# fzaiser/genfer

Hardware: AMD Instinct MI355X
Metric: TaylorPoly mul f64 GMAC/s (higher is better)
Workload: dtype f64

## Files before the change

### genfer_amd/__init__.py

```python
from __future__ import annotations

import ctypes
import os

os.environ.setdefault("HIP_FORCE_DEV_KERNARG", "1")

from . import series
from . import interval_series
from .taylor import USIZE_MAX, TaylorError, bind

_HERE = os.path.dirname(os.path.abspath(__file__))
LIB_PATH = os.path.join(_HERE, "csrc", "libgftaylor.so")

_lib = None
_classes = {}


def lib() -> ctypes.CDLL:
    global _lib
    if _lib is None:
        if not os.path.exists(LIB_PATH):
            raise ImportError(
                f"{LIB_PATH} is missing — build it with `make -C genfer_amd/csrc` "
                "(or `python -c 'import __graft_entry__ as g; g.build()'`). There is no CPU fallback."
# ... 86 lines not shown
    out, tj = ctypes.c_void_p(), ctypes.c_void_p()
    rc = H.gfh_run(source.encode(), flags.encode(), backend_lib.encode(), prefix.encode(), ctypes.byref(out), ctypes.byref(tj))
    text = ctypes.string_at(out).decode() if out else ""
    timings = json.loads(ctypes.string_at(tj).decode()) if tj else None
    if out:
        H.gfh_free(out)
    if tj:
        H.gfh_free(tj)
    return rc, text, timings


def run_sgcl(source: str, flags: str = ""):
    lib()
    prefix = "gfti_" if any(t in ("-b", "--bounds") for t in flags.split()) else "gft_"
    rc, text, timings = run_sgcl_with_backend(source, flags, LIB_PATH, prefix)
    if rc != 0:
        raise TaylorError(text)
    return text, timings


OP_STATS = ("linear_scans", "scalar_readbacks", "coefficient_readbacks", "tiled", "staged", "per_output", "host_tier_ops",
            "host_to_device_mirrors")
OP_STATS_EX = ("launches", "deferred_ops", "chains_materialised", "chain_addsub_launches", "launches_in_place", "shallow_products",
               "fused_horner_steps", "tiled_peeled", "unused_8", "riders", "fused_observe_adds", "scans_proven", "nested_adds",
               "graph_executions", "graph_recordings", "batch_launches", "batch_items", "graph_us")


def pool_stats() -> dict:
    a = (ctypes.c_size_t * 3)()
    lib().gft_pool_stats(a)
    return {"in_use": int(a[0]), "cached": int(a[1]), "peak": int(a[2])}


def op_stats() -> dict:
    L = lib()
    a, b = (ctypes.c_size_t * 8)(), (ctypes.c_size_t * 32)()
    L.gft_op_stats(a)
    n = min(L.gft_op_stats_ex(b, 32), 32)
    out = dict(zip(OP_STATS, (int(v) for v in a)))
    out.update(dict(zip(OP_STATS_EX, (int(v) for v in b[:n]))))
    return out


def _sz(seq):
    seq = [int(s) for s in seq]
    return (ctypes.c_size_t * max(len(seq), 1))(*seq)

# ... 41 lines not shown
```

### genfer_amd/csrc/gft_api.hip

```cpp
#include <hip/hip_runtime.h>
#include <dlfcn.h>
#include <rccl/rccl.h>

#include <algorithm>
#include <chrono>
#include <atomic>
#include <cmath>
#include <cstdio>
#include <cstring>
#include <deque>
#include <exception>
#include <functional>
#include <initializer_list>
#include <map>
#include <memory>
#include <tuple>
#include <stdexcept>
#include <string>
#include <vector>

#include "../../include/gftaylor.h"
#include "gft_kernels.hpp"
#include "gft_small_alloc.hpp"
#include "gft_host.hpp"
// ... 121 lines not shown
typedef SmallVecT<size_t> Dims;
typedef SmallVecT<long long> Shifts;

namespace {

struct Error : std::runtime_error {
    using std::runtime_error::runtime_error;
};

thread_local std::string g_err;

#define HIP_OK(call)                                                                                  \
    do {                                                                                              \
        hipError_t e_ = (call);                                                                       \
        if (e_ != hipSuccess)                                                                         \
            throw Error(std::string("HIP error: ") + hipGetErrorString(e_) + " in " #call);           \
    } while (0)

struct Runtime {
    bool ready = false;
    int device = -1;
    hipStream_t own_stream = nullptr;
    hipStream_t stream = nullptr;
    size_t stats_peeled = 0;
    size_t stats_side[4] = {0, 0, 0, 0};
    size_t stats_nz = 0;
    size_t stats_sum = 0;
    bool lazy_sum = true;
    bool nz_proofs = true;
    bool lazy_horner = true;
    bool batch_dag = true;
    bool lazy_observe = true;
    hipStream_t side = nullptr;
    hipEvent_t ev_main = nullptr, ev_bulk = nullptr;
    bool side_pending = false;
    bool recur_overlap = true;
    std::map<size_t, std::vector<void*>> free_blocks;
    size_t in_use = 0, cached = 0, peak = 0;
    size_t peak_total = 0;
    unsigned* d_flag = nullptr;
    double* d_scratch = nullptr;
    unsigned* d_wit = nullptr;
    double* h_pinned = nullptr;
    double* h_mail = nullptr;
    double* d_mail = nullptr;
    unsigned long long mail_seq = 0;
// ... 1035 lines not shown
    return guard_int([&] {
        HIP_OK(hipStreamSynchronize(R.stream));
        R.stream = s ? (hipStream_t)s : R.own_stream;
        return 0;
    });
}
void* gft_get_stream(void) { return (void*)R.stream; }
int gft_device(void) {
    return guard_int([&] { return R.device; });
}
int gft_synchronize(void) {
    return guard_int([&] {
        HIP_OK(hipStreamSynchronize(R.stream));
        return 0;
    });
}
const char* gft_last_error(void) { return g_err.c_str(); }
const char* gfti_last_error(void) { return g_err.c_str(); }
void gft_op_stats(size_t out[8]) {
    for (int i = 0; i < 8; ++i) out[i] = R.stats[i];
}
size_t gft_op_stats_ex(size_t* out, size_t cap) {
    const size_t v[18] = {(size_t)gft::g_launches, R.stats_ex[0], R.stats_ex[1], R.stats_ex[2], (size_t)gft::g_launches_in_place,
                          R.stats_shallow[0], R.stats_shallow[1], R.stats_peeled, R.stats_side[1], R.stats_side[2], R.stats_side[3], R.stats_nz, R.stats_sum,
                          g_dag_stats[0], g_dag_stats[1], g_dag_stats[2], g_dag_stats[3], g_dag_stats[4]};
    for (size_t i = 0; i < 18 && i < cap; ++i) out[i] = v[i];
    return 18;
}
void gft_pool_stats(size_t out[3]) {
    const size_t ws = staged_scratch_bytes() + R.conv_ws_bytes;
    out[0] = R.in_use + ws;
    out[1] = R.cached;
    R.peak_total = std::max(R.peak_total, R.in_use + ws);
    out[2] = R.peak_total;
}
int gft_event_record(int slot) {
    return guard_int([&] {
        if (slot < 0 || slot >= 64) throw Error("event slot out of range");
        HIP_OK(hipEventRecord(R.events[slot], R.stream));
        return 0;
    });
}
float gft_event_elapsed_ms(int a, int b) {
    try {
        require_ready();
        if (a < 0 || a >= 64 || b < 0 || b >= 64) throw Error("event slot out of range");
        HIP_OK(hipEventSynchronize(R.events[b]));
// ... 9 lines not shown
    std::string n = name ? name : "";
    if (n == "horner_loop_max") R.horner_loop_max = value < 0 ? 0 : (size_t)value;
    else if (n == "div_wavefront") R.div_wavefront = value != 0;
    else if (n == "exp_right") R.exp_right = value != 0;
    else if (n == "recur_overlap") R.recur_overlap = value != 0;
    else if (n == "defer") R.defer = value != 0;
    else if (n == "lazy_observe") R.lazy_observe = value != 0;
    else if (n == "batch_dag") R.batch_dag = value != 0;
    else if (n == "lazy_horner") R.lazy_horner = value != 0;
    else if (n == "nz_proofs") R.nz_proofs = value != 0;
    else if (n == "lazy_sum") R.lazy_sum = value != 0;
    else if (n == "async_launch") lq_configure(R.device, value != 0);
    else if (n == "trace_lq_report") lq_report();
    else if (n == "shallow_max_terms") R.shallow_max_terms = value < 0 ? 256 : (size_t)value;
    else if (n == "debug_fail_next_launch") g_fail_next_launch.store(value != 0 ? 1 : 0);
    else if (n == "tiled_min_macs") R.tiled_min_macs = value;
    else if (n == "conv_rb_min_macs") staged_set_rb_min_macs(value);
    else if (n == "conv_rb_pairs") staged_set_rb_pairs(value);
    else if (n == "conv_rb_pairs_cap") staged_set_rb_pairs_cap(value);
    else if (n == "conv_rb_pairs_lanes") staged_set_rb_pairs_lanes(value);
    else if (n == "shallow_pair_min") shallow_set_pair_min(value == -1.0 ? 4096.0 : value);
    else if (n == "tiled_tile") tiled_set_lane_tile((int)value);
    else if (n == "tiled_peel") tiled_set_peel((int)value);
    else if (n == "host_max_elems") R.host_max_elems = value < 0 ? Runtime::HOST_MAX_ELEMS_DEFAULT : (size_t)value;
    else if (n == "host_max_macs") R.host_max_macs = value < 0 ? Runtime::HOST_MAX_MACS_DEFAULT : value;
    else if (n == "series_form") R.series_force = (value == 1 || value == 2) ? (int)value : 0;
    else if (n == "dist_min_macs") dist_set_min_macs(value);
    else if (n == "dist_event_slot") dist_set_event_slot(value);
    else return -1;
    return 0;
}
int gft_set_conv_variant(int v) {
    R.conv_variant = v;
    return 0;
}
int gft_set_conv_mode(int mode) {
    if (mode < 0 || mode > 3) return -1;
    R.conv_mode = mode;
    return 0;
}

int gft_conv_raw(const double* x, const size_t* xshape, const double* y, const size_t* yshape, double* res,
                 const size_t* rshape, size_t ndim, size_t slab_lo, size_t slab_hi, int accumulate) {
    return guard_int([&] {
        typedef Ops<EF64> O;
        O::HV xv{const_cast<double*>(x), 0, dims(xshape, ndim)};
// ... 574 lines not shown
```

### genfer_amd/csrc/gft_conv_tiled.hip

```cpp
#include <algorithm>
#include <cstdlib>
#include <cstring>
#include <map>
#include <vector>

#include "gft_kernels.hpp"

namespace gft {

namespace {

struct TileSeg {
    unsigned u, a, b;
    unsigned step_begin, step_end;
    int dest;
};

struct RedTile {
    unsigned u, a, b;
    unsigned first, count;
    unsigned slot0;
};

struct TiledArgs {
    unsigned xU, x0, x1, xI;
    unsigned yU, y0, y1, yI;
    unsigned zU, z0, z1, zI;
    unsigned nx8, ny8;
    unsigned nxc, nyc, nb;
    unsigned P1;
    unsigned tsh;
    unsigned slab_axis;
    unsigned slab_lo, slab_hi;
    int accumulate;
    unsigned xcd_remap;
    unsigned cut;
    unsigned lim1;
    size_t zsU, zs0, zs1, zoff;
    const double* xp;
    const double* yp;
    double* z;
    double* ws;
    const TileSeg* segs;
    const unsigned* wg_begin;
    const RedTile* red;
    const unsigned* red_slots;
    const unsigned* guard;
    unsigned guard_epoch;
    unsigned char blk1[8], blk2[8];
};

typedef const double __attribute__((address_space(4))) * cptr_t;

#ifndef GFT_TILED_DEFAULT_VARIANT
// ... 175 lines not shown
    unsigned julo, n_ju, j0lo, n_j0, j1lo, n_j1;
};

__host__ __device__ inline TileGeom tile_geom(const TiledArgs& A, unsigned tsh, unsigned u, unsigned a, unsigned b) {
    TileGeom g;
    const unsigned T0 = 64u >> tsh, T1 = 1u << tsh;
    g.julo = (u + 1 > A.yU) ? (u + 1 - A.yU) : 0;
    unsigned juhi = (u + 1 < A.xU) ? (u + 1) : A.xU;
    g.n_ju = juhi > g.julo ? juhi - g.julo : 0;
    unsigned k0max = (T0 * a + T0 - 1 < A.z0 - 1) ? T0 * a + T0 - 1 : A.z0 - 1;
    g.j0lo = (T0 * a + 1 > A.y0) ? (T0 * a + 1 - A.y0) : 0;
    unsigned j0hi = (k0max + 1 < A.x0) ? (k0max + 1) : A.x0;
    if ((A.cut & 1u) && T0 * a + 1 < j0hi) j0hi = T0 * a + 1;
    g.n_j0 = j0hi > g.j0lo ? j0hi - g.j0lo : 0;
    unsigned k1max = (T1 * b + T1 - 1 < A.z1 - 1) ? T1 * b + T1 - 1 : A.z1 - 1;
    g.j1lo = (T1 * b + 1 > A.y1) ? (T1 * b + 1 - A.y1) : 0;
    unsigned j1hi = (k1max + 1 < A.x1) ? (k1max + 1) : A.x1;
    if ((A.cut & 2u) && T1 * b + 1 < j1hi) j1hi = T1 * b + 1;
    g.n_j1 = j1hi > g.j1lo ? j1hi - g.j1lo : 0;
    return g;
}

constexpr unsigned YPAD = 8;


template <int NW, int VAR, int TSH>
__global__ void __launch_bounds__(NW * 64, 4)
k_conv_tiled(TiledArgs A) {
    constexpr bool FAST = (VAR & 1) != 0;
    constexpr bool NO_WINDOW = (VAR & 64) != 0;
    constexpr bool PEEL = (VAR & 128) != 0;
    extern __shared__ double lds[];
    if (A.guard && *A.guard == A.guard_epoch) return;
    const unsigned tid = threadIdx.x;
    const unsigned lane = tid & 63u;
    const unsigned wave = __builtin_amdgcn_readfirstlane(tid >> 6);
    const unsigned tsh = TSH ? (unsigned)TSH : A.tsh, T1m = (1u << tsh) - 1u, T0 = 64u >> tsh;
    const unsigned l0 = lane >> tsh, l1 = lane & T1m;
    constexpr unsigned NT = NW * 64;

    const unsigned c1 = A.blk1[wave];
    const unsigned c2 = A.blk2[wave];
    const bool has1 = c1 != 0xffu;
    const bool has2 = c2 != 0xffu;

    const unsigned half_row = A.ny8 >> 1;
    const unsigned hr_magic = (1u << 24) / half_row + 1u;
    const size_t y_row_stride = A.ny8;
    const unsigned pf_s0 = (tid * hr_magic) >> 24, pf_col = tid - pf_s0 * half_row;
    const bool pf_mine = pf_s0 < T0;
    double* const lds_lane = lds + (size_t)(l0 << tsh) * A.P1 + YPAD;
    double* const lds_pf = lds + (size_t)(pf_s0 << tsh) * A.P1 + YPAD + 2 * pf_col;

    unsigned wg = blockIdx.x;
    if (A.xcd_remap) wg = (blockIdx.x & 7u) * (gridDim.x >> 3) + (blockIdx.x >> 3);
    const unsigned seg_begin = A.wg_begin[wg], seg_end = A.wg_begin[wg + 1];
    for (unsigned si = seg_begin; si < seg_end; ++si) {
        const TileSeg seg = A.segs[si];
        const unsigned u = seg.u, a = seg.a, b = seg.b;
        const TileGeom g = tile_geom(A, tsh, u, a, b);
        const unsigned k0 = T0 * a + l0, k1 = (b << tsh) + l1;
        bool lane_in = k0 < A.z0 && k1 < A.z1;
        if (A.slab_axis == 1) lane_in = lane_in && k0 >= A.slab_lo && k0 < A.slab_hi;
        else if (A.slab_axis == 2) lane_in = lane_in && k1 >= A.slab_lo && k1 < A.slab_hi;
        unsigned y1lim = A.y1;
        if (PEEL && A.lim1 && (k1 & ~7u) + 1u < y1lim) y1lim = (k1 & ~7u) + 1u;

        double acc1[8], acc2[8];
#pragma unroll
        for (int i = 0; i < 8; ++i) acc1[i] = acc2[i] = 0.0;

        unsigned tj1 = seg.step_begin % g.n_j1;
        unsigned t = seg.step_begin / g.n_j1;
        unsigned tj0 = t % g.n_j0;
        unsigned ju = g.julo + t / g.n_j0, j0 = g.j0lo + tj0, j1 = g.j1lo + tj1;
        unsigned steps_left = seg.step_end - seg.step_begin;
        const unsigned j1_end = g.j1lo + g.n_j1;

        while (steps_left) {
            const unsigned row_steps = steps_left < j1_end - j1 ? steps_left : j1_end - j1;
            const double* ybase = A.yp + (size_t)(u - ju) * A.y0 * A.y1 * y_row_stride;
            if (!NO_WINDOW) {
                __syncthreads();
                for (unsigned p = tid; p < 64 * half_row; p += NT) {
                    unsigned row = (p * hr_magic) >> 24, col = p - row * half_row;
                    unsigned s0 = row >> tsh, s1 = row & T1m;
                    int R0 = (int)(T0 * a + s0) - (int)j0;
                    int R1 = (int)((b << tsh) + s1) - (int)j1;
                    if (R0 >= 0 && R0 < (int)A.y0 && R1 >= 0 && R1 < (int)A.y1) {
                        const double2 v = *reinterpret_cast<const double2*>(
                            ybase + ((size_t)R0 * A.y1 + (size_t)R1) * y_row_stride + 2 * col);
                        double* d = lds + ((s0 << tsh) + ((unsigned)R1 & T1m)) * A.P1 + YPAD + 2 * col;
                        d[0] = v.x;
                        d[1] = v.y;
                    }
                }
                __syncthreads();
            }
            cptr_t xr = (cptr_t)(A.xp + (((size_t)ju * A.x0 + j0) * A.x1 + j1) * A.nx8);
            const bool valid0 = lane_in && j0 <= k0 && (k0 - j0) < A.y0;
            int d1 = (int)k1 - (int)j1;
            int R1n = (int)(b << tsh) - (int)j1 - 1;
            const int pf_R0 = (int)(T0 * a + pf_s0) - (int)j0;
            const bool pf_row = pf_mine && pf_R0 >= 0 && pf_R0 < (int)A.y0;
            const double* pf_src = ybase + ((ptrdiff_t)pf_R0 * (ptrdiff_t)A.y1 + R1n) * (ptrdiff_t)y_row_stride + 2 * pf_col;

            for (unsigned rs = row_steps; rs > 0; --rs) {
                const bool last = rs == 1;
                const bool do_pf = !NO_WINDOW && !last && R1n >= 0 && R1n < (int)A.y1;
                double2 pf;
                if (do_pf && pf_row) pf = *reinterpret_cast<const double2*>(pf_src);

                if (valid0 && (unsigned)d1 < (PEEL ? y1lim : A.y1)) {
                    const double* yrow = lds_lane + (size_t)((unsigned)d1 & T1m) * A.P1;
                    if constexpr (FAST && (VAR & 8)) {
                        if (has1) block_fast_gen<VAR>(acc1, c1, xr, yrow, A.nxc, A.nyc);
                        if (has2) block_fast_gen<VAR>(acc2, c2, xr, yrow, A.nxc, A.nyc);
                    } else if constexpr (FAST) {
                        if (has1) block_fast<VAR>(acc1, c1, xr, yrow);
                        if (has2) block_fast<VAR>(acc2, c2, xr, yrow);
                    } else {
                        if (has1) block_mac<VAR>(acc1, c1, xr, yrow, A.nxc, A.nyc);
                        if (has2) block_mac<VAR>(acc2, c2, xr, yrow, A.nxc, A.nyc);
                    }
                }

                if (!last && !NO_WINDOW) {
                    __syncthreads();
                    if (do_pf && pf_row) {
                        double* d = lds_pf + (size_t)((unsigned)R1n & T1m) * A.P1;
                        d[0] = pf.x;
                        d[1] = pf.y;
                    }
                    __syncthreads();
                }
                xr += A.nx8;
                d1 -= 1;
                R1n -= 1;
                pf_src -= y_row_stride;
            }
            steps_left -= row_steps;
            j1 = g.j1lo;
            if (j0 + 1 < g.j0lo + g.n_j0) j0++;
            else {
                j0 = g.j0lo;
                ju++;
            }
        }

        if (seg.dest < 0) {
            if (lane_in) {
                double* zrow = A.z + (((size_t)u * A.z0 + k0) * A.z1 + k1) * A.zI;
                if constexpr (PEEL) zrow = A.z + A.zoff + (size_t)u * A.zsU + (size_t)k0 * A.zs0 + (size_t)k1 * A.zs1;
                if (has1) {
#pragma unroll
                    for (int r = 0; r < 8; ++r) {
                        unsigned k2 = 8 * c1 + r;
                        if (k2 < A.zI) zrow[k2] = A.accumulate ? zrow[k2] + acc1[r] : acc1[r];
                    }
                }
                if (has2) {
// ... 251 lines not shown
    plan_cache().clear();
    plan_generation()++;
    arena().head = 0;
}

int num_cus() {
    static int n = 0;
    if (!n) {
        int dev = 0;
        (void)hipGetDevice(&dev);
        hipDeviceProp_t p;
        if (hipGetDeviceProperties(&p, dev) == hipSuccess) n = p.multiProcessorCount;
        if (n <= 0) n = 256;
    }
    return n;
}

struct PeelSpec {
    unsigned role = 0;
    unsigned cut = 0, lim1 = 0;
    size_t zsU = 0, zs0 = 0, zs1 = 0, zoff = 0;
};

int& tiled_force_tsh() {
    static int v = 0;
    return v;
}

unsigned pick_lane_tile(const TiledArgs& T) {
    auto axis_eff = [](unsigned T, unsigned nx, unsigned ny, unsigned nz) {
        double useful = 0, issued = 0;
        for (unsigned t = 0; t * T < nz; ++t) {
            const unsigned kmax = std::min(T * t + T - 1, nz - 1);
            const unsigned jlo = T * t + 1 > ny ? T * t + 1 - ny : 0, jhi = std::min(kmax + 1, nx);
            if (jhi > jlo) issued += (double)(jhi - jlo) * T;
            for (unsigned k = T * t; k <= kmax; ++k) {
                const unsigned lo = k + 1 > ny ? k + 1 - ny : 0, hi = std::min(k + 1, nx);
                if (hi > lo) useful += hi - lo;
            }
        }
        return issued > 0 ? useful / issued : 0.0;
    };
    const int force = tiled_force_tsh();
    if (force >= 3 && force <= 6) return (unsigned)force;
    double best = -1.0;
    unsigned best_tsh = 3;
// ... 20 lines not shown
    }
    auto cost = [&](unsigned c) {
        unsigned n = 0;
        for (unsigned xc = 0; xc <= c && xc < T.nxc; ++xc)
            if (c - xc < T.nyc) n++;
        return n;
    };
    unsigned simd_load[4] = {0, 0, 0, 0}, wave_load[8] = {0}, wave_cnt[8] = {0};
    for (unsigned i = 0; i < T.nb; ++i) {
        unsigned c = T.nb - 1 - i;
        int best = -1;
        for (unsigned w = 0; w < NW; ++w) {
            if (wave_cnt[w] >= 2) continue;
            if (best < 0) { best = (int)w; continue; }
            unsigned sb = simd_load[best % 4], sw = simd_load[w % 4];
            if (sw < sb || (sw == sb && wave_load[w] < wave_load[best])) best = (int)w;
        }
        if (wave_cnt[best] == 0) T.blk1[best] = (unsigned char)c;
        else T.blk2[best] = (unsigned char)c;
        wave_cnt[best]++;
        wave_load[best] += cost(c);
        simd_load[best % 4] += cost(c);
    }
}

bool canonicalise(const ConvArgs& a, const Variant& V, const PeelSpec& ps, Plan& P) {
    TiledArgs& T = P.base;
    std::memset(&T, 0, sizeof(T));
    if (a.slab_axis < 0 || a.slab_axis >= a.nd - 1) return false;
    if (a.nd == 2) {
        T.xU = T.yU = T.zU = 1;
        T.x0 = T.y0 = T.z0 = 1;
        T.x1 = a.xs[0]; T.xI = a.xs[1];
        T.y1 = a.ys[0]; T.yI = a.ys[1];
        T.z1 = a.zs[0]; T.zI = a.zs[1];
        T.slab_axis = 2;
    } else if (a.nd == 3) {
        T.xU = T.yU = T.zU = 1;
        T.x0 = a.xs[0]; T.x1 = a.xs[1]; T.xI = a.xs[2];
        T.y0 = a.ys[0]; T.y1 = a.ys[1]; T.yI = a.ys[2];
        T.z0 = a.zs[0]; T.z1 = a.zs[1]; T.zI = a.zs[2];
        T.slab_axis = 1 + (unsigned)a.slab_axis;
    } else if (a.nd == 4) {
        T.xU = a.xs[0]; T.x0 = a.xs[1]; T.x1 = a.xs[2]; T.xI = a.xs[3];
        T.yU = a.ys[0]; T.y0 = a.ys[1]; T.y1 = a.ys[2]; T.yI = a.ys[3];
        T.zU = a.zs[0]; T.z0 = a.zs[1]; T.z1 = a.zs[2]; T.zI = a.zs[3];
// ... 2 lines not shown
        return false;
    }
    if (T.zI > 128 || T.xI > T.zI || T.yI > T.zI) return false;
    if (a.j0_min != 0 || a.j0_excl != 0 || a.j0_desc != 0) return false;
    T.nx8 = (T.xI + 7) / 8 * 8;
    T.ny8 = (T.yI + 7) / 8 * 8;
    T.nxc = T.nx8 / 8;
    T.nyc = T.ny8 / 8;
    T.nb = (T.zI + 7) / 8;
    T.P1 = V.b128 ? T.ny8 + YPAD + 2 : T.ny8 + YPAD + 1;
    T.tsh = pick_lane_tile(T);
    T.cut = ps.cut;
    T.lim1 = ps.lim1;
    if (ps.role >= 2) {
        T.zsU = ps.zsU; T.zs0 = ps.zs0; T.zs1 = ps.zs1; T.zoff = ps.zoff;
    } else {
        T.zsU = (size_t)T.z0 * T.z1 * T.zI; T.zs0 = (size_t)T.z1 * T.zI; T.zs1 = T.zI; T.zoff = 0;
    }
    T.slab_lo = a.slab_lo;
    T.slab_hi = a.slab_hi;
    T.accumulate = a.accumulate;
    unsigned npairs = (T.nb + 1) / 2;
    P.NW = npairs <= 1 ? 1 : (npairs <= 2 ? 2 : (npairs <= 4 ? 4 : 8));
    P.lds_bytes = (size_t)64 * T.P1 * sizeof(double);
    assign_blocks(T, P.NW);
    return true;
}

struct PlanTables {
    std::vector<TileSeg> segs;
    std::vector<unsigned> wg_begin;
    std::vector<RedTile> red;
    std::vector<unsigned> red_slots;
    bool slots_consecutive = true;
};

bool cut_ranges(Plan& P, PlanTables& tb) {
    const TiledArgs& T = P.base;
    const unsigned TT0 = 64u >> T.tsh, TT1 = 1u << T.tsh;
    struct TileInfo { unsigned u, a, b; unsigned long long steps; };
    std::vector<TileInfo> tiles;
    unsigned u_lo = 0, u_hi = T.zU, a_lo = 0, a_hi = (T.z0 + TT0 - 1) / TT0, b_lo = 0, b_hi = (T.z1 + TT1 - 1) / TT1;
    if (T.slab_axis == 0) {
        u_lo = T.slab_lo;
        u_hi = T.slab_hi;
    } else if (T.slab_axis == 1) {
        a_lo = T.slab_lo / TT0;
        a_hi = (T.slab_hi + TT0 - 1) / TT0;
    } else {
        b_lo = T.slab_lo / TT1;
        b_hi = (T.slab_hi + TT1 - 1) / TT1;
    }
    unsigned long long S = 0;
    for (unsigned u = u_lo; u < u_hi; ++u)
        for (unsigned aa = a_lo; aa < a_hi; ++aa)
            for (unsigned bb = b_lo; bb < b_hi; ++bb) {
                TileGeom g = tile_geom(T, T.tsh, u, aa, bb);
                unsigned long long st = (unsigned long long)g.n_ju * g.n_j0 * g.n_j1;
                if (st == 0 || st > 0xffffffffull) return false;
                tiles.push_back({u, aa, bb, st});
                S += st;
            }
    if (tiles.empty()) return false;
    unsigned wg_per_cu = std::min<unsigned>(16u / P.NW, (unsigned)(160 * 1024 / P.lds_bytes));
    if (wg_per_cu < 1) wg_per_cu = 1;
    unsigned long long n_wg = (unsigned long long)num_cus() * wg_per_cu;
    const unsigned long long per_slot = S / n_wg;
    const unsigned long long fit = per_slot / 190;
    n_wg *= fit >= 8 ? 8u : (fit >= 4 ? 4u : (fit >= 2 ? 2u : 1u));
    constexpr unsigned long long MIN_UNITS = 64;
    const unsigned long long step_units = (unsigned long long)T.nb * (T.nb + 1) / 2 + 3;
    const unsigned long long min_steps =
        std::max<unsigned long long>(1, (MIN_UNITS + 20ull * T.nb + step_units / 2) / step_units);
    if (n_wg > S / min_steps) n_wg = std::max<unsigned long long>(1, S / min_steps);
    P.n_wg = (unsigned)n_wg;

    tb.wg_begin.assign(P.n_wg + 1, 0);
    std::vector<std::vector<unsigned>> tile_slots(tiles.size());
    std::vector<int> tile_direct(tiles.size(), 0);
    unsigned n_slots = 0;
    size_t ti = 0;
    unsigned long long tile_start = 0;
    for (unsigned w = 0; w < P.n_wg; ++w) {
        unsigned long long lo = S * w / n_wg, hi = S * (w + 1) / n_wg;
        tb.wg_begin[w] = (unsigned)tb.segs.size();
        unsigned long long pos = lo;
        while (pos < hi) {
            while (pos >= tile_start + tiles[ti].steps) {
// ... 54 lines not shown
        }
        off += al(bytes);
        return d;
    };
    T.segs = (const TileSeg*)put(tb.segs.data(), b_segs);
    T.wg_begin = (const unsigned*)put(tb.wg_begin.data(), b_wg);
    T.red = (const RedTile*)put(tb.red.data(), b_red);
    T.red_slots = (const unsigned*)put(tb.red_slots.data(), b_rs);
    if (tb.slots_consecutive) T.red_slots = nullptr;
    if (hbase && hipMemcpyAsync(base, hbase, off, hipMemcpyHostToDevice, st) != hipSuccess) return false;
    return true;
}

bool build_plan(const ConvArgs& a, const Variant& V, const PeelSpec& ps, Plan& P, hipStream_t st) {
    PlanTables tb;
    return canonicalise(a, V, ps, P) && cut_ranges(P, tb) && upload_tables(P, tb, st);
}

template <int NW, int VAR, int TSH>
void launch_main_t(hipStream_t st, const Plan& P, const TiledArgs& T) {
    static bool attr_set = false;
    if (!attr_set) {
        (void)hipFuncSetAttribute(reinterpret_cast<const void*>(&k_conv_tiled<NW, VAR, TSH>),
                                  hipFuncAttributeMaxDynamicSharedMemorySize, 160 * 1024);
        attr_set = true;
    }
    GFT_LAUNCH((k_conv_tiled<NW, VAR, TSH>), dim3(P.n_wg), dim3(NW * 64), P.lds_bytes, st, T);
}
template <int NW, int VAR>
void launch_main_nw(hipStream_t st, const Plan& P, const TiledArgs& T) {
    if (T.tsh == 3) launch_main_t<NW, VAR, 3>(st, P, T);
    else launch_main_t<NW, VAR, 0>(st, P, T);
}
template <int VAR>
void launch_main(hipStream_t st, const Plan& P, const TiledArgs& T) {
    switch (P.NW) {
        case 1: launch_main_nw<1, VAR>(st, P, T); break;
        case 2: launch_main_nw<2, VAR>(st, P, T); break;
        case 4: launch_main_nw<4, VAR>(st, P, T); break;
        default: launch_main_nw<8, VAR>(st, P, T); break;
    }
}

}

void tiled_pad_rows_f64(hipStream_t st, const double* in, double* out, size_t rows, unsigned len, unsigned P, unsigned B) {
    size_t tot = rows * P * B;
// ... 2 lines not shown
                       len, P, B);
}
void tiled_fold_rows_f64(hipStream_t st, const double* zt, double* z, size_t rows, size_t row_lo, size_t row_hi, unsigned Pz,
                         unsigned B, unsigned zI, int accumulate, const unsigned* guard, unsigned epoch) {
    size_t tot = (row_hi - row_lo) * zI;
    if (!tot) return;
    GFT_LAUNCH(k_fold_rows, dim3((unsigned)std::min<size_t>((tot + 255) / 256, 4096)), dim3(256), 0, st, zt, z, rows,
                       row_lo, row_hi, Pz, B, zI, accumulate, guard, epoch);
}

void tiled_set_lane_tile(int tsh) { tiled_force_tsh() = tsh; }

namespace {

int& tiled_peel_mode() {
    static int v = GFT_TILED_PEEL_DEFAULT;
    return v;
}

const Plan* cached_plan(const ConvArgs& a, const Variant& V, const PeelSpec& ps, hipStream_t st) {
    PlanKey key;
    std::memset(&key, 0, sizeof(key));
    if (a.nd < 2 || a.nd > 4) return nullptr;
    key.v[0] = (unsigned)a.nd | ((unsigned)a.slab_axis << 8) | ((unsigned)tiled_force_tsh() << 16);
    for (int i = 0; i < a.nd; ++i) {
        key.v[1 + i] = a.xs[i];
        key.v[5 + i] = a.ys[i];
        key.v[9 + i] = a.zs[i];
    }
    key.v[13] = a.slab_lo;
    key.v[14] = a.slab_hi;
    key.v[15] = (unsigned)a.accumulate;
    key.v[16] = (unsigned)(a.j0_min | (a.j0_excl << 8) | (a.j0_desc << 16));
    key.v[17] = V.b128;
    key.v[18] = ps.role | (ps.cut << 4) | (ps.lim1 << 8);
    auto& cache = plan_cache();
    auto it = cache.find(key);
    if (it == cache.end()) {
        Plan P;
        if (cache.size() >= 1024) reset_plan_cache(st);
        if (!build_plan(a, V, ps, P, st)) return nullptr;
        it = cache.emplace(key, P).first;
    }
    return &it->second;
}

bool launch_plan(hipStream_t st, const Plan& P, TiledArgs T, const Variant& V) {
// ... 55 lines not shown
    T.guard = nf_flag;
    T.guard_epoch = nf_epoch;
}

bool peel_applies(const ConvArgs& a, const Variant& V) {
    const int mode = tiled_peel_mode();
    if (mode == 0) return false;
    if (a.nd != 3 || a.slab_axis != 0 || a.slab_lo != 0 || a.slab_hi != a.zs[0]) return false;
    if (a.j0_min || a.j0_excl || a.j0_desc) return false;
    for (int i = 0; i < 3; ++i)
        if (a.xs[i] != a.zs[i] || a.ys[i] != a.zs[i]) return false;
    const unsigned n0 = a.zs[0], n1 = a.zs[1];
    if (n0 % 8 || n1 % 8 || n0 < 16 || n1 < 16 || a.zs[2] > 128) return false;
    if (!V.fast || !V.b128 || V.compact || V.peel || V.other) return false;
    TiledArgs T;
    std::memset(&T, 0, sizeof(T));
    T.x0 = T.y0 = T.z0 = n0;
    T.x1 = T.y1 = T.z1 = n1;
    if (pick_lane_tile(T) != 3) return false;
    return mode == 1 || (n0 >= PEEL_MIN_EXTENT && n1 >= PEEL_MIN_EXTENT && a.zs[2] >= PEEL_MIN_INNER);
}

int conv_tiled_peel(hipStream_t st, const double* x, const double* y, double* z, const ConvArgs& a, const Variant& V, void* ws,
                    size_t ws_bytes, size_t* ws_needed, unsigned* nf_flag, unsigned nf_epoch, bool* guarded) {
    const unsigned n0 = a.zs[0], n1 = a.zs[1], nI = a.zs[2];
    ConvArgs l0, l1;
    std::memset(&l0, 0, sizeof(l0));
    l0.nd = 4;
    l0.slab_lo = 0;
    l0.slab_hi = 7;
    l0.accumulate = 1;
    l1 = l0;
    Variant VL = V;
    VL.peel = true;
    const unsigned s0x[4] = {7, 1, n1, nI}, s0y[4] = {7, n0 / 8, n1, nI}, s1x[4] = {7, 1, n0, nI}, s1y[4] = {7, n1 / 8, n0, nI};
    for (int i = 0; i < 4; ++i) {
        l0.xs[i] = s0x[i]; l0.ys[i] = l0.zs[i] = s0y[i];
        l1.xs[i] = s1x[i]; l1.ys[i] = l1.zs[i] = s1y[i];
    }
    PeelSpec pm, p0, p1;
    pm.role = 1; pm.cut = 3;
    p0.role = 2; p0.zsU = (size_t)n1 * nI; p0.zs0 = 8 * p0.zsU; p0.zs1 = nI; p0.zoff = p0.zsU;
    p1.role = 3; p1.lim1 = 1; p1.zsU = nI; p1.zs0 = 8 * (size_t)nI; p1.zs1 = (size_t)n1 * nI; p1.zoff = nI;
    Plan PM, P0, P1;
    for (int attempt = 0;; ++attempt) {
        const unsigned long long gen = plan_generation();
        const Plan* q = cached_plan(a, V, pm, st);
        if (!q) return -1;
        PM = *q;
        if (!(q = cached_plan(l0, VL, p0, st))) return -1;
        P0 = *q;
        if (!(q = cached_plan(l1, VL, p1, st))) return -1;
        P1 = *q;
        if (gen == plan_generation()) break;
        if (attempt) return -1;
    }
    const TiledArgs& B = PM.base;
    if (B.tsh != 3) return -1;
    const size_t n8 = B.nx8;
    const Operands o = operand_layout(B, std::max(PM.n_slots, std::max(P0.n_slots, P1.n_slots)), x, y, a.operands_slack);
    const size_t e_w0 = (size_t)7 * (n0 / 8) * n1 * n8, e_s1 = (size_t)7 * n0 * n8, e_w1 = (size_t)7 * (n1 / 8) * n0 * n8;
    auto al = [](size_t v) { return (v + 255) / 256 * 256; };
    const size_t o_w0 = o.end, o_s1 = o_w0 + al(e_w0 * sizeof(double)), o_w1 = o_s1 + al((e_s1 + 8) * sizeof(double)),
                 need = o_w1 + al(e_w1 * sizeof(double)) + 256;
    if (ws && ws_bytes < need) return -1;
    if (ws_needed) *ws_needed = need;
    if (guarded) *guarded = !o.inplace;
    if (!ws) return 1;

    char* wb = (char*)ws;
    double *w0 = (double*)(wb + o_w0), *s1 = (double*)(wb + o_s1), *w1 = (double*)(wb + o_w1);
    TiledArgs T = B;
    bind_operands(st, o, x, y, wb, nf_flag, nf_epoch, T);
    {
        const size_t tot = e_w0 + e_s1 + e_w1;
        GFT_LAUNCH(k_pack_peel, dim3((unsigned)std::min<size_t>((tot + 255) / 256, 4096)), dim3(256), 0, st, x, y, w0, s1, w1, n0, n1,
                   nI, (unsigned)n8);
    }
    T.z = z;
    if (!launch_plan(st, PM, T, V)) return 0;
    TiledArgs T0 = P0.base, T1 = P1.base;
    T0.ws = T1.ws = T.ws;
    T0.z = T1.z = z;
    T0.guard = T1.guard = T.guard;
    T0.guard_epoch = T1.guard_epoch = T.guard_epoch;
    T0.xp = T.yp;
    T0.yp = w0;
    T1.xp = s1;
    T1.yp = w1;
    return launch_plan(st, P0, T0, VL) && launch_plan(st, P1, T1, VL) ? 1 : 0;
}

}

void tiled_set_peel(int mode) { tiled_peel_mode() = mode < 0 ? -1 : (mode ? 1 : 0); }

bool conv_tiled_f64(hipStream_t st, const double* x, const double* y, double* z, const ConvArgs& a, void* ws, size_t ws_bytes,
                    size_t* ws_needed, unsigned* nf_flag, unsigned nf_epoch, bool* guarded, bool* peeled) {
    bool compact_operands = false;
    if (a.nd >= 2 && a.nd <= 4) {
        const unsigned nb = (a.zs[a.nd - 1] + 7) / 8;
        compact_operands = (a.xs[a.nd - 1] + 7) / 8 < nb || (a.ys[a.nd - 1] + 7) / 8 < nb;
    }
    const Variant V = decode_variant(a.variant, compact_operands);
    if (peeled) *peeled = false;
    if (peel_applies(a, V)) {
        const int r = conv_tiled_peel(st, x, y, z, a, V, ws, ws_bytes, ws_needed, nf_flag, nf_epoch, guarded);
        if (r >= 0) {
            if (peeled) *peeled = r == 1;
            return r == 1;
        }
    }
    const Plan* P = cached_plan(a, V, PeelSpec(), st);
    if (!P) return false;
    const Operands o = operand_layout(P->base, P->n_slots, x, y, a.operands_slack);
    const size_t need = o.end + 256;
    if (guarded) *guarded = !o.inplace;
    if (ws_needed) *ws_needed = need;
    if (!ws) return true;
    if (ws_bytes < need) return false;
    TiledArgs T = P->base;
    bind_operands(st, o, x, y, (char*)ws, nf_flag, nf_epoch, T);
    T.z = z;
    return launch_plan(st, *P, T, V);
}

}
```

### genfer_amd/csrc/gft_kernels.hpp

```cpp
#pragma once
#include <hip/hip_runtime.h>

#include <cstddef>
#include <cstdint>
#include <vector>

#include "gft_elem.hpp"
#include "gft_launch.hpp"
#include "gft_wavefront_plan.hpp"

namespace gft {

constexpr int MAXD = 12;

struct Shape {
    int nd;
    unsigned d[MAXD];
};

struct DView {
    double* p;
    size_t plane;
    Shape sh;
};
// ... 273 lines not shown
                       unsigned log_k = 0, double* res2 = nullptr, size_t r2_plane = 0);
    static void recur_wavefront(hipStream_t st, const WfPlan& plan, const double* xs, size_t x_plane, const double* ys, size_t y_plane,
                                double* res, size_t r_plane, double* qb, size_t q_plane, unsigned* flags);
    static void factor_table(hipStream_t st, int op, unsigned n, unsigned len, const double* m, size_t m_plane,
                             double* tab, size_t tab_plane);
    static void sum_axis(hipStream_t st, const double* in, size_t in_plane, unsigned outer, unsigned len,
                         unsigned inner, size_t axis_stride_outer, double* out, size_t out_plane, int mode);
    static void any_zero(hipStream_t st, const double* p, size_t plane, size_t n, unsigned* state, const Mailbox& mb);
    static void zero_pattern(hipStream_t st, const double* p, size_t plane, const Shape& sh, size_t n, unsigned* state, const Mailbox& mb);
    static void count_neq(hipStream_t st, const double* a, size_t a_plane, const double* b, size_t b_plane,
                          size_t n, unsigned* count);
    static void conv_naive(hipStream_t st, const double* x, size_t x_plane, const double* y, size_t y_plane,
                           double* z, size_t z_plane, const ConvArgs& a);
    static bool conv_shallow(hipStream_t st, const double* x, size_t x_plane, const double* y, size_t y_plane, double* out,
                             size_t out_plane, const ConvArgs& a, const ConvEpi& e);
    static bool conv_line(hipStream_t st, const double* x, size_t x_plane, const double* y, size_t y_plane, double* z, size_t z_plane,
                          const ConvArgs& a);
};

enum SumMode { SUM_SEQ = 0, SUM_UNROLL8 = 1, SUM_WAVE = 2 };

bool conv_tiled_f64(hipStream_t st, const double* x, const double* y, double* z, const ConvArgs& a, void* ws,
                    size_t ws_bytes, size_t* ws_needed, unsigned* nf_flag, unsigned nf_epoch, bool* guarded = nullptr,
                    bool* peeled = nullptr);

template <class E>
bool conv_pairs(hipStream_t st, const double* x, size_t xp, const double* y, size_t yp, double* z, size_t zp, const ConvArgs& a, double max_macs);
void staged_set_rb_min_macs(double v);
void staged_set_rb_pairs(double v);
void staged_set_rb_pairs_cap(double bytes);
void shallow_set_pair_min(double v);
void staged_set_rb_pairs_lanes(double v);
size_t staged_scratch_bytes();
void staged_release_scratch();
void dwf_release_orders();
void tiled_set_lane_tile(int tsh);
void tiled_set_peel(int mode);
void tiled_pad_rows_f64(hipStream_t st, const double* in, double* out, size_t rows, unsigned len, unsigned P, unsigned B);
void tiled_fold_rows_f64(hipStream_t st, const double* zt, double* z, size_t rows, size_t row_lo, size_t row_hi, unsigned Pz,
                         unsigned B, unsigned zI, int accumulate, const unsigned* guard, unsigned epoch);

template <class E>
bool conv_staged(hipStream_t st, const double* x, size_t x_plane, const double* y, size_t y_plane, double* z,
                 size_t z_plane, const ConvArgs& a, bool force);

}
```

### genfer_amd/csrc/gft_ops_product.inc

```

    static void conv(const HV& x, const HV& y, const HV& z, size_t slab_lo, size_t slab_hi, bool accumulate,
                     bool slab_mode, int j0_min, int j0_excl, int j0_desc) {
        Dims keep = collapse_mask({&z.shape}, slab_mode);
        Dims xs = pick(x.shape, keep), ys = pick(y.shape, keep), zs = pick(z.shape, keep);
        if (zs.size() > (size_t)MAXD) throw Error("tensor rank exceeds GFT MAXD after collapsing");
        ConvArgs a;
        std::memset(&a, 0, sizeof(a));
        a.nd = (int)zs.size();
        Dims xst = c_strides(xs), yst = c_strides(ys), zst = c_strides(zs);
        for (int i = 0; i < a.nd; ++i) {
            a.xs[i] = (unsigned)xs[i];
            a.ys[i] = (unsigned)ys[i];
            a.zs[i] = (unsigned)zs[i];
            a.xstr[i] = xst[i];
            a.ystr[i] = yst[i];
            a.zstr[i] = zst[i];
        }
        if (!z.shape.empty() && slab_hi <= slab_lo) return;
        const bool axis0_kept = !keep.empty() && keep[0] == 0;
        if (a.nd == 0) {
            a.slab_lo = 0;
            a.slab_hi = 1;
        } else if (!axis0_kept) {
            a.slab_lo = 0;
// ... 79 lines not shown
        }
        if (want_tiled && ash.nd > 4 && !ash.accumulate && ash.zs[ash.nd - 1] <= 128 && conv_tiled_high_rank(x, y, z, a, ash, tx, ty, tz)) return;
        if (want_tiled) {
            ConvArgs at = ash;
            unsigned B = 0;
            const bool split = plan_inner_split(ash, at, &B);
            if (split) at.operands_slack = 0;
            size_t need = 0;
            bool ok = true;
            if (R.conv_mode == 0) {
                double macs = 1.0;
                for (int i = 0; i < ash.nd; ++i) {
                    double f = 0.5 * (double)ash.zs[i] * (double)std::min(ash.xs[i], ash.ys[i]);
                    if (i == 0 && ash.slab_hi - ash.slab_lo < ash.zs[0]) f = (double)(ash.slab_hi - ash.slab_lo) * std::min(ash.xs[0], ash.ys[0]);
                    macs *= f;
                }
                const double tmin = R.tiled_min_override >= 0 ? R.tiled_min_override : R.tiled_min_macs;
                if (macs < tmin * (split ? 10.0 : (ash.nd == 2 ? 4.0 : 1.0))) ok = false;
            }
            if (ok) ok = conv_tiled_f64(R.stream, tx, ty, tz, at, nullptr, 0, &need, nullptr, 0);
            if (ok) {
                R.ensure_conv_ws(need);
                unsigned* flag = R.next_nf_epoch();
                bool guarded = true;
                if (!split) {
                    bool peeled = false;
                    if (!conv_tiled_f64(R.stream, tx, ty, tz, ash, R.conv_ws, R.conv_ws_bytes, &need, flag, R.nf_epoch, &guarded, &peeled))
                        throw Error("tiled convolution launch failed");
                    if (peeled) R.stats_peeled++;
                } else {
                    const ConvArgs& a = ash;
                    const double* xsrc = tx;
                    const double* ysrc = ty;
                    double* zdst = tz;
                    const int nd = a.nd;
                    size_t xrows = 1, yrows = 1, zrows = 1, zrows_per0 = 1;
                    for (int i = 0; i + 1 < nd; ++i) {
                        xrows *= a.xs[i];
                        yrows *= a.ys[i];
                        zrows *= a.zs[i];
                        if (i > 0) zrows_per0 *= a.zs[i];
                    }
                    const unsigned Px = at.xs[0], Py = at.ys[0], Pz = at.zs[0], RI = 2 * B - 1;
                    Rc<Buf> xt = alloc_doubles(xrows * Px * B), yt = alloc_doubles(yrows * Py * B);
                    Rc<Buf> zt = alloc_doubles(zrows * Pz * RI);
                    tiled_pad_rows_f64(R.stream, xsrc, xt->p, xrows, a.xs[nd - 1], Px, B);
                    tiled_pad_rows_f64(R.stream, ysrc, yt->p, yrows, a.ys[nd - 1], Py, B);
                    if (!conv_tiled_f64(R.stream, xt->p, yt->p, zt->p, at, R.conv_ws, R.conv_ws_bytes, &need, flag, R.nf_epoch))
                        throw Error("tiled convolution launch failed");
                    size_t per0 = nd == 2 ? 1 : zrows_per0;
                    tiled_fold_rows_f64(R.stream, zt->p, zdst, zrows, a.slab_lo * per0, a.slab_hi * per0, Pz, B, a.zs[nd - 1],
                                        a.accumulate, flag, R.nf_epoch);
                }
                R.stats[3]++;
                if (!guarded) return;
                a.guard = flag;
                a.guard_epoch = R.nf_epoch;
                if (!conv_staged<E>(R.stream, x.p, x.plane, y.p, y.plane, z.p, z.plane, a, false))
                    K<E>::conv_naive(R.stream, x.p, x.plane, y.p, y.plane, z.p, z.plane, a);
                return;
            }
            if (R.conv_mode == 2) throw Error("conv_mode=2 (tiled) requested but the shape is not supported by the tiled kernel");
        }
        if (R.conv_mode == 0 || R.conv_mode == 3) {
            if (conv_staged<E>(R.stream, x.p, x.plane, y.p, y.plane, z.p, z.plane, a, R.conv_mode == 3)) {
                R.stats[4]++;
                return;
            }
        }
        R.stats[5]++;
        K<E>::conv_naive(R.stream, x.p, x.plane, y.p, y.plane, z.p, z.plane, a);
    }

    static bool conv_tiled_high_rank(const HV& x, const HV& y, const HV& z, const ConvArgs& a, const ConvArgs& ash, const double* tx,
                                     const double* ty, double* tz) {
        const int extra = ash.nd - 4;
        ConvArgs sub;
// ... 161 lines not shown
```

Baseline: 29780.

## Add spare LDS ring slot to tiled conv window to drop a barrier

The tiled convolution's y-window in LDS becomes a ring of T1+1 rows instead of T1, indexed by a rotating slot counter. With the spare slot, the prefetched next row can be written without first waiting for all lanes to finish reading, so one of the two __syncthreads per step is removed. Ring length is picked automatically: the spare slot is used only when it does not reduce the number of resident workgroups per CU, and an option can force it on or off. The cost is extra LDS, modulo slot arithmetic in the inner loop, and a new stats counter.

```diff
diff --git a/genfer_amd/__init__.py b/genfer_amd/__init__.py
--- a/genfer_amd/__init__.py
+++ b/genfer_amd/__init__.py
@@ -132,7 +132,7 @@
 OP_STATS = ("linear_scans", "scalar_readbacks", "coefficient_readbacks", "tiled", "staged", "per_output", "host_tier_ops",
             "host_to_device_mirrors")
 OP_STATS_EX = ("launches", "deferred_ops", "chains_materialised", "chain_addsub_launches", "launches_in_place", "shallow_products",
-               "fused_horner_steps", "tiled_peeled", "unused_8", "riders", "fused_observe_adds", "scans_proven", "nested_adds",
+               "fused_horner_steps", "tiled_peeled", "tiled_ring_spare", "riders", "fused_observe_adds", "scans_proven", "nested_adds",
                "graph_executions", "graph_recordings", "batch_launches", "batch_items", "graph_us")
 
 
diff --git a/genfer_amd/csrc/gft_api.hip b/genfer_amd/csrc/gft_api.hip
--- a/genfer_amd/csrc/gft_api.hip
+++ b/genfer_amd/csrc/gft_api.hip
@@ -167,6 +167,7 @@
     int device = -1;
     hipStream_t own_stream = nullptr;
     hipStream_t stream = nullptr;
+    size_t stats_ring_spare = 0;
     size_t stats_peeled = 0;
     size_t stats_side[4] = {0, 0, 0, 0};
     size_t stats_nz = 0;
@@ -1248,7 +1249,7 @@
 }
 size_t gft_op_stats_ex(size_t* out, size_t cap) {
     const size_t v[18] = {(size_t)gft::g_launches, R.stats_ex[0], R.stats_ex[1], R.stats_ex[2], (size_t)gft::g_launches_in_place,
-                          R.stats_shallow[0], R.stats_shallow[1], R.stats_peeled, R.stats_side[1], R.stats_side[2], R.stats_side[3], R.stats_nz, R.stats_sum,
+                          R.stats_shallow[0], R.stats_shallow[1], R.stats_peeled, R.stats_ring_spare, R.stats_side[2], R.stats_side[3], R.stats_nz, R.stats_sum,
                           g_dag_stats[0], g_dag_stats[1], g_dag_stats[2], g_dag_stats[3], g_dag_stats[4]};
     for (size_t i = 0; i < 18 && i < cap; ++i) out[i] = v[i];
     return 18;
@@ -1304,6 +1305,7 @@
     else if (n == "shallow_pair_min") shallow_set_pair_min(value == -1.0 ? 4096.0 : value);
     else if (n == "tiled_tile") tiled_set_lane_tile((int)value);
     else if (n == "tiled_peel") tiled_set_peel((int)value);
+    else if (n == "tiled_ring") tiled_set_ring((int)value);
     else if (n == "host_max_elems") R.host_max_elems = value < 0 ? Runtime::HOST_MAX_ELEMS_DEFAULT : (size_t)value;
     else if (n == "host_max_macs") R.host_max_macs = value < 0 ? Runtime::HOST_MAX_MACS_DEFAULT : value;
     else if (n == "series_form") R.series_force = (value == 1 || value == 2) ? (int)value : 0;
diff --git a/genfer_amd/csrc/gft_conv_tiled.hip b/genfer_amd/csrc/gft_conv_tiled.hip
--- a/genfer_amd/csrc/gft_conv_tiled.hip
+++ b/genfer_amd/csrc/gft_conv_tiled.hip
@@ -30,6 +30,7 @@
     unsigned nxc, nyc, nb;
     unsigned P1;
     unsigned tsh;
+    unsigned ring;
     unsigned slab_axis;
     unsigned slab_lo, slab_hi;
     int accumulate;
@@ -251,6 +252,7 @@
 }
 
 constexpr unsigned YPAD = 8;
+constexpr size_t LDS_PER_CU = 160 * 1024;
 
 
 template <int NW, int VAR, int TSH>
@@ -278,8 +280,10 @@
     const size_t y_row_stride = A.ny8;
     const unsigned pf_s0 = (tid * hr_magic) >> 24, pf_col = tid - pf_s0 * half_row;
     const bool pf_mine = pf_s0 < T0;
-    double* const lds_lane = lds + (size_t)(l0 << tsh) * A.P1 + YPAD;
-    double* const lds_pf = lds + (size_t)(pf_s0 << tsh) * A.P1 + YPAD + 2 * pf_col;
+    const unsigned RL = A.ring;
+    const bool spare = RL != T1m + 1u;
+    double* const lds_lane = lds + (size_t)(l0 * RL) * A.P1 + YPAD;
+    double* const lds_pf = lds + (size_t)(pf_s0 * RL) * A.P1 + YPAD + 2 * pf_col;
 
     unsigned wg = blockIdx.x;
     if (A.xcd_remap) wg = (blockIdx.x & 7u) * (gridDim.x >> 3) + (blockIdx.x >> 3);
@@ -309,6 +313,9 @@
         while (steps_left) {
             const unsigned row_steps = steps_left < j1_end - j1 ? steps_left : j1_end - j1;
             const double* ybase = A.yp + (size_t)(u - ju) * A.y0 * A.y1 * y_row_stride;
+            int R1n = (int)(b << tsh) - (int)j1 - 1;
+            int sn = R1n % (int)RL;
+            if (sn < 0) sn += (int)RL;
             if (!NO_WINDOW) {
                 __syncthreads();
                 for (unsigned p = tid; p < 64 * half_row; p += NT) {
@@ -319,7 +326,9 @@
                     if (R0 >= 0 && R0 < (int)A.y0 && R1 >= 0 && R1 < (int)A.y1) {
                         const double2 v = *reinterpret_cast<const double2*>(
                             ybase + ((size_t)R0 * A.y1 + (size_t)R1) * y_row_stride + 2 * col);
-                        double* d = lds + ((s0 << tsh) + ((unsigned)R1 & T1m)) * A.P1 + YPAD + 2 * col;
+                        unsigned slot = (unsigned)sn + 1u + s1;
+                        if (slot >= RL) slot -= RL;
+                        double* d = lds + (s0 * RL + slot) * A.P1 + YPAD + 2 * col;
                         d[0] = v.x;
                         d[1] = v.y;
                     }
@@ -329,7 +338,6 @@
             cptr_t xr = (cptr_t)(A.xp + (((size_t)ju * A.x0 + j0) * A.x1 + j1) * A.nx8);
             const bool valid0 = lane_in && j0 <= k0 && (k0 - j0) < A.y0;
             int d1 = (int)k1 - (int)j1;
-            int R1n = (int)(b << tsh) - (int)j1 - 1;
             const int pf_R0 = (int)(T0 * a + pf_s0) - (int)j0;
             const bool pf_row = pf_mine && pf_R0 >= 0 && pf_R0 < (int)A.y0;
             const double* pf_src = ybase + ((ptrdiff_t)pf_R0 * (ptrdiff_t)A.y1 + R1n) * (ptrdiff_t)y_row_stride + 2 * pf_col;
@@ -340,32 +348,34 @@
                 double2 pf;
                 if (do_pf && pf_row) pf = *reinterpret_cast<const double2*>(pf_src);
 
-                if (valid0 && (unsigned)d1 < (PEEL ? y1lim : A.y1)) {
-                    const double* yrow = lds_lane + (size_t)((unsigned)d1 & T1m) * A.P1;
-                    if constexpr (FAST && (VAR & 8)) {
-                        if (has1) block_fast_gen<VAR>(acc1, c1, xr, yrow, A.nxc, A.nyc);
-                        if (has2) block_fast_gen<VAR>(acc2, c2, xr, yrow, A.nxc, A.nyc);
-                    } else if constexpr (FAST) {
-                        if (has1) block_fast<VAR>(acc1, c1, xr, yrow);
-                        if (has2) block_fast<VAR>(acc2, c2, xr, yrow);
-                    } else {
-                        if (has1) block_mac<VAR>(acc1, c1, xr, yrow, A.nxc, A.nyc);
-                        if (has2) block_mac<VAR>(acc2, c2, xr, yrow, A.nxc, A.nyc);
-                    }
+                const bool active = valid0 && (unsigned)d1 < (PEEL ? y1lim : A.y1);
+                unsigned slot = (unsigned)sn + 1u + l1;
+                if (slot >= RL) slot -= RL;
+                const double* yrow = lds_lane + (size_t)slot * A.P1;
+                auto block = [&](double (&acc)[8], unsigned c) {
+                    if constexpr (FAST && (VAR & 8)) block_fast_gen<VAR>(acc, c, xr, yrow, A.nxc, A.nyc);
+                    else if constexpr (FAST) block_fast<VAR>(acc, c, xr, yrow);
+                    else block_mac<VAR>(acc, c, xr, yrow, A.nxc, A.nyc);
+                };
+                const bool refill = do_pf && pf_row;
+                double* const pf_dst = lds_pf + (size_t)sn * A.P1;
+                if (active) {
+                    if (has1) block(acc1, c1);
+                    if (has2) block(acc2, c2);
                 }
 
                 if (!last && !NO_WINDOW) {
-                    __syncthreads();
-                    if (do_pf && pf_row) {
-                        double* d = lds_pf + (size_t)((unsigned)R1n & T1m) * A.P1;
-                        d[0] = pf.x;
-                        d[1] = pf.y;
+                    if (!spare) __syncthreads();
+                    if (refill) {
+                        pf_dst[0] = pf.x;
+                        pf_dst[1] = pf.y;
                     }
                     __syncthreads();
                 }
                 xr += A.nx8;
                 d1 -= 1;
                 R1n -= 1;
+                sn = sn ? sn - 1 : (int)RL - 1;
                 pf_src -= y_row_stride;
             }
             steps_left -= row_steps;
@@ -663,6 +673,11 @@
     size_t zsU = 0, zs0 = 0, zs1 = 0, zoff = 0;
 };
 
+int& tiled_ring_mode() {
+    static int v = -1;
+    return v;
+}
+
 int& tiled_force_tsh() {
     static int v = 0;
     return v;
@@ -729,6 +744,19 @@
         wave_load[best] += cost(c);
         simd_load[best % 4] += cost(c);
     }
+}
+
+size_t window_bytes(const TiledArgs& T, unsigned ring) { return (size_t)(64u >> T.tsh) * ring * T.P1 * sizeof(double); }
+unsigned resident_wgs(size_t lds_bytes, unsigned NW) {
+    return std::max(1u, std::min<unsigned>(16u / NW, (unsigned)(LDS_PER_CU / lds_bytes)));
+}
+unsigned ring_length(const TiledArgs& T, unsigned NW) {
+    const unsigned T1 = 1u << T.tsh;
+    const int mode = tiled_ring_mode();
+    const size_t with = window_bytes(T, T1 + 1);
+    if (mode == 0 || with > LDS_PER_CU) return T1;
+    if (mode == 1) return T1 + 1;
+    return resident_wgs(with, NW) == resident_wgs(window_bytes(T, T1), NW) ? T1 + 1 : T1;
 }
 
 bool canonicalise(const ConvArgs& a, const Variant& V, const PeelSpec& ps, Plan& P) {
@@ -777,7 +805,8 @@
     T.accumulate = a.accumulate;
     unsigned npairs = (T.nb + 1) / 2;
     P.NW = npairs <= 1 ? 1 : (npairs <= 2 ? 2 : (npairs <= 4 ? 4 : 8));
-    P.lds_bytes = (size_t)64 * T.P1 * sizeof(double);
+    T.ring = ring_length(T, P.NW);
+    P.lds_bytes = window_bytes(T, T.ring);
     assign_blocks(T, P.NW);
     return true;
 }
@@ -817,8 +846,7 @@
                 S += st;
             }
     if (tiles.empty()) return false;
-    unsigned wg_per_cu = std::min<unsigned>(16u / P.NW, (unsigned)(160 * 1024 / P.lds_bytes));
-    if (wg_per_cu < 1) wg_per_cu = 1;
+    const unsigned wg_per_cu = resident_wgs(P.lds_bytes, P.NW);
     unsigned long long n_wg = (unsigned long long)num_cus() * wg_per_cu;
     const unsigned long long per_slot = S / n_wg;
     const unsigned long long fit = per_slot / 190;
@@ -919,7 +947,7 @@
     static bool attr_set = false;
     if (!attr_set) {
         (void)hipFuncSetAttribute(reinterpret_cast<const void*>(&k_conv_tiled<NW, VAR, TSH>),
-                                  hipFuncAttributeMaxDynamicSharedMemorySize, 160 * 1024);
+                                  hipFuncAttributeMaxDynamicSharedMemorySize, (int)LDS_PER_CU);
         attr_set = true;
     }
     GFT_LAUNCH((k_conv_tiled<NW, VAR, TSH>), dim3(P.n_wg), dim3(NW * 64), P.lds_bytes, st, T);
@@ -968,7 +996,7 @@
     PlanKey key;
     std::memset(&key, 0, sizeof(key));
     if (a.nd < 2 || a.nd > 4) return nullptr;
-    key.v[0] = (unsigned)a.nd | ((unsigned)a.slab_axis << 8) | ((unsigned)tiled_force_tsh() << 16);
+    key.v[0] = (unsigned)a.nd | ((unsigned)a.slab_axis << 8) | ((unsigned)tiled_force_tsh() << 16) | ((unsigned)(tiled_ring_mode() + 1) << 24);
     for (int i = 0; i < a.nd; ++i) {
         key.v[1 + i] = a.xs[i];
         key.v[5 + i] = a.ys[i];
@@ -1070,7 +1098,7 @@
 }
 
 int conv_tiled_peel(hipStream_t st, const double* x, const double* y, double* z, const ConvArgs& a, const Variant& V, void* ws,
-                    size_t ws_bytes, size_t* ws_needed, unsigned* nf_flag, unsigned nf_epoch, bool* guarded) {
+                    size_t ws_bytes, size_t* ws_needed, unsigned* nf_flag, unsigned nf_epoch, bool* guarded, bool* ring_spare) {
     const unsigned n0 = a.zs[0], n1 = a.zs[1], nI = a.zs[2];
     ConvArgs l0, l1;
     std::memset(&l0, 0, sizeof(l0));
@@ -1114,6 +1142,7 @@
     if (ws && ws_bytes < need) return -1;
     if (ws_needed) *ws_needed = need;
     if (guarded) *guarded = !o.inplace;
+    if (ring_spare) *ring_spare = B.ring != 8;
     if (!ws) return 1;
 
     char* wb = (char*)ws;
@@ -1142,9 +1171,10 @@
 }
 
 void tiled_set_peel(int mode) { tiled_peel_mode() = mode < 0 ? -1 : (mode ? 1 : 0); }
+void tiled_set_ring(int mode) { tiled_ring_mode() = mode < 0 ? -1 : (mode ? 1 : 0); }
 
 bool conv_tiled_f64(hipStream_t st, const double* x, const double* y, double* z, const ConvArgs& a, void* ws, size_t ws_bytes,
-                    size_t* ws_needed, unsigned* nf_flag, unsigned nf_epoch, bool* guarded, bool* peeled) {
+                    size_t* ws_needed, unsigned* nf_flag, unsigned nf_epoch, bool* guarded, bool* peeled, bool* ring_spare) {
     bool compact_operands = false;
     if (a.nd >= 2 && a.nd <= 4) {
         const unsigned nb = (a.zs[a.nd - 1] + 7) / 8;
@@ -1152,8 +1182,9 @@
     }
     const Variant V = decode_variant(a.variant, compact_operands);
     if (peeled) *peeled = false;
+    if (ring_spare) *ring_spare = false;
     if (peel_applies(a, V)) {
-        const int r = conv_tiled_peel(st, x, y, z, a, V, ws, ws_bytes, ws_needed, nf_flag, nf_epoch, guarded);
+        const int r = conv_tiled_peel(st, x, y, z, a, V, ws, ws_bytes, ws_needed, nf_flag, nf_epoch, guarded, ring_spare);
         if (r >= 0) {
             if (peeled) *peeled = r == 1;
             return r == 1;
@@ -1164,6 +1195,7 @@
     const Operands o = operand_layout(P->base, P->n_slots, x, y, a.operands_slack);
     const size_t need = o.end + 256;
     if (guarded) *guarded = !o.inplace;
+    if (ring_spare) *ring_spare = P->base.ring != 1u << P->base.tsh;
     if (ws_needed) *ws_needed = need;
     if (!ws) return true;
     if (ws_bytes < need) return false;
diff --git a/genfer_amd/csrc/gft_kernels.hpp b/genfer_amd/csrc/gft_kernels.hpp
--- a/genfer_amd/csrc/gft_kernels.hpp
+++ b/genfer_amd/csrc/gft_kernels.hpp
@@ -319,7 +319,7 @@
 
 bool conv_tiled_f64(hipStream_t st, const double* x, const double* y, double* z, const ConvArgs& a, void* ws,
                     size_t ws_bytes, size_t* ws_needed, unsigned* nf_flag, unsigned nf_epoch, bool* guarded = nullptr,
-                    bool* peeled = nullptr);
+                    bool* peeled = nullptr, bool* ring_spare = nullptr);
 
 template <class E>
 bool conv_pairs(hipStream_t st, const double* x, size_t xp, const double* y, size_t yp, double* z, size_t zp, const ConvArgs& a, double max_macs);
@@ -333,6 +333,7 @@
 void dwf_release_orders();
 void tiled_set_lane_tile(int tsh);
 void tiled_set_peel(int mode);
+void tiled_set_ring(int mode);
 void tiled_pad_rows_f64(hipStream_t st, const double* in, double* out, size_t rows, unsigned len, unsigned P, unsigned B);
 void tiled_fold_rows_f64(hipStream_t st, const double* zt, double* z, size_t rows, size_t row_lo, size_t row_hi, unsigned Pz,
                          unsigned B, unsigned zI, int accumulate, const unsigned* guard, unsigned epoch);
diff --git a/genfer_amd/csrc/gft_ops_product.inc b/genfer_amd/csrc/gft_ops_product.inc
--- a/genfer_amd/csrc/gft_ops_product.inc
+++ b/genfer_amd/csrc/gft_ops_product.inc
@@ -125,10 +125,11 @@
             if (ok) {
                 R.ensure_conv_ws(need);
                 unsigned* flag = R.next_nf_epoch();
-                bool guarded = true;
+                bool guarded = true, ring_spare = false;
                 if (!split) {
                     bool peeled = false;
-                    if (!conv_tiled_f64(R.stream, tx, ty, tz, ash, R.conv_ws, R.conv_ws_bytes, &need, flag, R.nf_epoch, &guarded, &peeled))
+                    if (!conv_tiled_f64(R.stream, tx, ty, tz, ash, R.conv_ws, R.conv_ws_bytes, &need, flag, R.nf_epoch, &guarded, &peeled,
+                                        &ring_spare))
                         throw Error("tiled convolution launch failed");
                     if (peeled) R.stats_peeled++;
                 } else {
@@ -149,13 +150,15 @@
                     Rc<Buf> zt = alloc_doubles(zrows * Pz * RI);
                     tiled_pad_rows_f64(R.stream, xsrc, xt->p, xrows, a.xs[nd - 1], Px, B);
                     tiled_pad_rows_f64(R.stream, ysrc, yt->p, yrows, a.ys[nd - 1], Py, B);
-                    if (!conv_tiled_f64(R.stream, xt->p, yt->p, zt->p, at, R.conv_ws, R.conv_ws_bytes, &need, flag, R.nf_epoch))
+                    if (!conv_tiled_f64(R.stream, xt->p, yt->p, zt->p, at, R.conv_ws, R.conv_ws_bytes, &need, flag, R.nf_epoch, nullptr, nullptr,
+                                        &ring_spare))
                         throw Error("tiled convolution launch failed");
                     size_t per0 = nd == 2 ? 1 : zrows_per0;
                     tiled_fold_rows_f64(R.stream, zt->p, zdst, zrows, a.slab_lo * per0, a.slab_hi * per0, Pz, B, a.zs[nd - 1],
                                         a.accumulate, flag, R.nf_epoch);
                 }
                 R.stats[3]++;
+                if (ring_spare) R.stats_ring_spare++;
                 if (!guarded) return;
                 a.guard = flag;
                 a.guard_epoch = R.nf_epoch;
```

Result: slower. 29220 (-1.9%).
